# NVlabs/curobo

Measured on NVIDIA H100. Metric: rollout_cost_grad_evals_per_sec, higher is better.
Workload: dtype f32

## Files before the change

curobo_b200/csrc/cb200_kernels.cu:

```cuda
#include <cuda_runtime.h>
#include <stdio.h>
#include <stdlib.h>
#include <string.h>

#include <algorithm>
#include <cmath>
#include <vector>

#include "../../include/curobo_b200.h"
#include "cb200_blob.h"
#include "cb200_bspline.cuh"
#include "cb200_dynamics.cuh"
#include "cb200_dynamics_tile.cuh"
#include "cb200_launch.h"
#include "cb200_math.cuh"
#include "cb200_mesh.cuh"
#include "cb200_warp.cuh"

using namespace cb200;

namespace {

constexpr int kWarpsPerCta = 8;
#ifndef CB200_MINB
// ... 139 lines not shown
    bound_cost(qd, lim[d], lim[D + d], c.cspace_activation[0], wb[0], cost, gp);
    bound_cost(v, lim[2 * D + d], lim[3 * D + d], c.cspace_activation[1], wb[1], cost, gv);
    bound_cost(ac, lim[4 * D + d], lim[5 * D + d], c.cspace_activation[2], wb[2], cost, ga);
    bound_cost(jk, lim[6 * D + d], lim[7 * D + d], c.cspace_activation[3], wb[3], cost, gj);
    cspace_target_term(a, b, h, d, D, qd, cost, gp);
    l2_reg(v, wr[0], cost, gv);
    l2_reg(ac, wr[1], cost, ga);
    l2_reg(jk, wr[2], cost, gj);
    if (a.grad_vel) a.grad_vel[idx] = gv;
    if (a.grad_acc) a.grad_acc[idx] = ga;
    if (a.grad_jerk) a.grad_jerk[idx] = gj;
  }
  return cost;
}

template <bool SPLINE>
__device__ __forceinline__ void row_phase_a(const FusedArgs &a, const RobotView &rv, const EvalSmem &es, int lane, int e,
                                            int b, int h, float &cs_cost, float &pose_c) {
  const cb200_rollout_cfg &cfg = a.cfg;
  const int D = rv.D, S = rv.S, L = rv.L;
  cs_cost = 0.0f;
  #pragma unroll 1
  for (int d = lane; d < D; d += 32) {
    const bspline::State4 st = load_row_state<SPLINE>(a, e, b, h, d, D);
    es.qv[d] = st.p;
    float gp;
    const float c = cspace_dof(a, rv, e, b, h, d, st, gp);
    es.gqv[d] = gp;
    cs_cost += c;
    if (a.cspace_cost) a.cspace_cost[(size_t)e * D + d] = c;
  }
  __syncwarp();
  warp_fk(rv, es, lane);
  warp_spheres(rv, es, lane, a.robot_spheres ? reinterpret_cast<float4 *>(a.robot_spheres) + (size_t)e * S : nullptr,
               row_sphere_cfg(a, b, S));
  pose_c = 0.0f;
  const bool do_pose = (a.goal_position != nullptr);
  #pragma unroll 1
  for (int t = lane; t < L; t += 32) {
    const float *T = es.cumul + 12 * rv.tool_map[t];
    const V3 p = mk3(T[3], T[7], T[11]);
    const Q4 qt = quat_from_transform(T);
    if (a.link_pos) {
      float *o = a.link_pos + ((size_t)e * L + t) * 3;
      o[0] = p.x;
      o[1] = p.y;
      o[2] = p.z;
    }
    if (a.link_quat) *reinterpret_cast<float4 *>(a.link_quat + ((size_t)e * L + t) * 4) = make_float4(qt.w, qt.x, qt.y, qt.z);
    float *pg = es.pose_g + 8 * t;
    pg[0] = pg[1] = pg[2] = pg[4] = pg[5] = pg[6] = 0.0f;
    if (do_pose) {
      const int gi = a.idxs_goal ? __ldg(a.idxs_goal + b) : 0;
      const bool term = !(h < a.H - 1 && a.H > 1);
// ... 7 lines not shown
      const V3 om = quat_grad_to_omega(qt, po.gq_w, po.gq_x, po.gq_y, po.gq_z);
      pg[0] = po.g_pos.x;
      pg[1] = po.g_pos.y;
      pg[2] = po.g_pos.z;
      pg[4] = om.x;
      pg[5] = om.y;
      pg[6] = om.z;
      pose_c += po.pos_cost + po.rot_cost;
      if (a.pose_cost) {
        a.pose_cost[((size_t)e * L + t) * 2] = po.pos_cost;
        a.pose_cost[((size_t)e * L + t) * 2 + 1] = po.rot_cost;
      }
      if (a.pose_goalset_idx) a.pose_goalset_idx[(size_t)e * L + t] = po.goal_idx;
    }
  }
  __syncwarp();
}

struct RowB1 {
  float self_c, fmax, scene_c;
  int bi, bj, nnz;
};

template <bool SWEEP, int SCENE, bool CULL2 = true>
__device__ __forceinline__ RowB1 row_phase_b1(const FusedArgs &a, const RobotView &rv, const EvalSmem &es, int lane, int e,
                                              int b, const float4 *prev_sph, const float4 *next_sph) {
  const cb200_rollout_cfg &cfg = a.cfg;
  const int S = rv.S;
  RowB1 r{0.0f, 0.0f, 0.0f, 0, 0, 0};
  if (cfg.self_weight > 0.0f && rv.P > 0) {
    r.fmax = (rv.n_lp > 0) ? warp_self_collision_tiles<true, CULL2>(rv, es, lane, r.bi, r.bj)
                           : warp_self_collision_pairs(es.gsph, rv.pairs, rv.P, lane, r.bi, r.bj);
    r.self_c = (r.fmax > 0.0f) ? 0.5f * cfg.self_weight * r.fmax : 0.0f;
  }
  if (a.self_cost && lane == 0) a.self_cost[e] = r.self_c;
  __syncwarp();
  const bool do_scene = SCENE != 0 && cfg.scene_weight > 0.0f;
  const int env = (a.env_query_idx != nullptr) ? __ldg(a.env_query_idx + b) : 0;
  const float sdt = (SWEEP && cfg.use_speed_metric && (a.dt != nullptr || a.spl.knots != nullptr))
                        ? (a.spl.knots != nullptr ? __ldg(a.spl.traj_dt + __ldg(a.spl.goal_idx)) : __ldg(a.dt))
                        : 0.0f;
  int ce = 0, ncub = 0;
  bool cull = false;
  if ((SCENE & 1) && do_scene) {
    ce = env < a.cuboids.num_envs ? env : 0;
    ncub = a.cuboids.count[ce];
    if (ncub > a.cuboids.max_n) ncub = a.cuboids.max_n;
    cull = !SWEEP && rv.n_lp > 0 && ncub <= 32;
    if (cull) {
#pragma unroll 1
      for (int ca = lane; ca < rv.n_cl; ca += 32) {
        const float4 cb = rv.cl_bound_scene[ca];
        uint32_t mask = 0u;
        if (cb.w >= 0.0f) {
          const float *Tk = es.cumul + 12 * rv.cl_link[ca];
          const V3 cw = mk3(Tk[0] * cb.x + Tk[1] * cb.y + Tk[2] * cb.z + Tk[3], Tk[4] * cb.x + Tk[5] * cb.y + Tk[6] * cb.z + Tk[7],
                            Tk[8] * cb.x + Tk[9] * cb.y + Tk[10] * cb.z + Tk[11]);
#pragma unroll 1
          for (int i = 0; i < ncub; ++i) {
            const int kk = ce * a.cuboids.max_n + i;
            if (a.cuboids.enable[kk] != 1) continue;
            const ObsFrame f = load_obs_frame(a.cuboids.inv_pose + 8 * kk);
            const SdfGrad sg = cuboid_sdf_grad(to_obstacle(f, cw), ldgf(a.cuboids.dims + 4 * kk), ldgf(a.cuboids.dims + 4 * kk + 1),
                                               ldgf(a.cuboids.dims + 4 * kk + 2));
            if (sg.sdf < cb.w + cfg.scene_activation) mask |= (1u << i);
          }
        }
        es.cmask[ca] = mask;
      }
      __syncwarp();
    }
  }
#pragma unroll 1
  for (int s = lane; s < S; s += 32) {
    V3 g = mk3(0, 0, 0);
    float c = 0.0f;
    if (do_scene) {
      const float4 sp = es.sph[s];
      const V3 cen = mk3(sp.x, sp.y, sp.z);
      if (!SWEEP) {
        if (sp.w >= 0.0f) {
          if (SCENE & 1) {
            uint32_t m = cull ? es.cmask[rv.sph_cl[s]] : 0xffffffffu;
            const float radj = sp.w + cfg.scene_activation;
#pragma unroll 1
            for (int i = 0; i < ncub && m != 0u; ++i) {
              if (cull && !((m >> i) & 1u)) continue;
              if (cull) m &= ~(1u << i);
              const int kk = ce * a.cuboids.max_n + i;
// ... 23 lines not shown
        }
        if (next_sph != nullptr) {
          const float4 t = next_sph[s];
          nx = mk3(t.x, t.y, t.z);
        }
        c = sphere_scene_swept<SCENE>(cen, sp.w, cfg.scene_activation, cfg.scene_weight, prev_sph != nullptr, pv,
                                      next_sph != nullptr, nx, a.cuboids, a.voxels, env, g);
        if (cfg.use_speed_metric && prev_sph != nullptr && next_sph != nullptr) speed_metric(pv, cen, nx, sdt, c, g);
      }
    }
    es.gsph[s] = make_float4(g.x, g.y, g.z, 0.0f);
    r.nnz += (g.x != 0.0f || g.y != 0.0f || g.z != 0.0f) ? 1 : 0;
    r.scene_c += c;
    if (a.scene_cost) a.scene_cost[(size_t)e * S + s] = c;
  }
  __syncwarp();
  r.nnz = (int)__reduce_add_sync(kFull, (unsigned)r.nnz) + 2;
  return r;
}

template <bool SMALL = false>
__device__ __forceinline__ void row_phase_b2(const FusedArgs &a, const RobotView &rv, const EvalSmem &es,
                                             const unsigned char *smem_blob, int lane, int e, const RowB1 &r,
                                             float cs_cost, float pose_c) {
  if (r.fmax > 0.0f && lane == 0) {
    const float4 pi = es.sph[r.bi], pj = es.sph[r.bj];
    const float w = a.cfg.self_weight;
    float4 gi = es.gsph[r.bi], gj = es.gsph[r.bj];
    const float gx = w * (pj.x - pi.x), gy = w * (pj.y - pi.y), gz = w * (pj.z - pi.z);
    gi.x += gx;
    gi.y += gy;
    gi.z += gz;
    gj.x -= gx;
    gj.y -= gy;
    gj.z -= gz;
    es.gsph[r.bi] = gi;
    es.gsph[r.bj] = gj;
  }
  __syncwarp();
  float *gq = a.grad_q + (size_t)e * rv.D;
  if (!warp_fk_backward_sparse<SMALL>(rv, es, lane, gq, r.nnz)) warp_fk_backward_cold(smem_blob, a.blob, es.cumul, lane, gq);
  const float tot = warp_sum(cs_cost + pose_c + r.scene_c) + r.self_c;
  if (lane == 0) a.cost[e] = tot;
  __syncwarp();
}

#ifdef CB200_OOL_PHASES
struct PhaseAOut {
  float cs_cost, pose_c;
};
static __device__ __noinline__ PhaseAOut phase_a_ool(const FusedArgs *a, const unsigned char *smem, float *base, int lane,
                                                     int e, int b, int h) {
  const RobotView rv = make_robot_view(smem, a->blob);
  const EvalSmem es = carve_eval_smem(base, rv.nl, rv.D, rv.S, rv.L, rv.n_cl);
  PhaseAOut o;
  row_phase_a<false>(*a, rv, es, lane, e, b, h, o.cs_cost, o.pose_c);
  return o;
}
template <int SCENE>
static __device__ __noinline__ RowB1 phase_b1_ool(const FusedArgs *a, const unsigned char *smem, float *base, int lane, int e,
                                                  int b) {
  const RobotView rv = make_robot_view(smem, a->blob);
  const EvalSmem es = carve_eval_smem(base, rv.nl, rv.D, rv.S, rv.L, rv.n_cl);
  return row_phase_b1<false, SCENE>(*a, rv, es, lane, e, b, nullptr, nullptr);
}
static __device__ __noinline__ void phase_b2_ool(const FusedArgs *a, const unsigned char *smem, float *base, int lane, int e,
                                                 RowB1 r, float cs_cost, float pose_c) {
  const RobotView rv = make_robot_view(smem, a->blob);
  const EvalSmem es = carve_eval_smem(base, rv.nl, rv.D, rv.S, rv.L, rv.n_cl);
  row_phase_b2(*a, rv, es, smem, lane, e, r, cs_cost, pose_c);
}
#endif

template <int SCENE, bool SPLINE, int MINB = CB200_MINB>
__global__ void __launch_bounds__(kWarpsPerCta * 32, MINB) rollout_fused_kernel(const __grid_constant__ FusedArgs a) {
  CB200_EXTERN_SHARED __align__(128) unsigned char smem[];
  __shared__ unsigned long long mbar;
  stage_blob_to_smem(smem, a.blob, (uint32_t)a.blob_smem_bytes, &mbar);
  const int warp = threadIdx.x >> 5, lane = threadIdx.x & 31, nwarps = blockDim.x >> 5;
  float *base = reinterpret_cast<float *>(smem + a.blob_smem_bytes) + (size_t)warp * a.eval_floats;
  const int N = a.B * a.H;
  const int stride = gridDim.x * nwarps;
  int e = blockIdx.x * nwarps + warp;
  while (e < N) {
    int b = e, h = 0;
    if (a.H != 1) {
      b = e / a.H;
      h = e - b * a.H;
    }
#ifndef CB200_OOL_PHASES
    const RobotView rv = make_robot_view(smem, a.blob);
    const EvalSmem es = carve_eval_smem(base, rv.nl, rv.D, rv.S, rv.L, rv.n_cl);
    float cs_cost = 0.0f, pose_c = 0.0f;
    row_phase_a<SPLINE>(a, rv, es, lane, e, b, h, cs_cost, pose_c);
    const RowB1 r = row_phase_b1<false, SCENE, MINB != 3>(a, rv, es, lane, e, b, nullptr, nullptr);
    row_phase_b2<MINB == 3>(a, rv, es, smem, lane, e, r, cs_cost, pose_c);
#else
    const PhaseAOut pa = phase_a_ool(&a, smem, base, lane, e, b, h);
    const RowB1 r = phase_b1_ool<SCENE>(&a, smem, base, lane, e, b);
    phase_b2_ool(&a, smem, base, lane, e, r, pa.cs_cost, pa.pose_c);
#endif
    if (a.work_counter != nullptr) {
      int nxt = 0;
      if (lane == 0) nxt = stride + atomicAdd(a.work_counter, 1);
      e = __shfl_sync(kFull, nxt, 0);
    } else {
      e += stride;
    }
  }
  if (a.work_counter != nullptr && lane == 0) {
    __threadfence();
    if (atomicAdd(a.work_counter + 1, 1) == stride - 1) {
      a.work_counter[0] = 0;
      a.work_counter[1] = 0;
    }
  }
}

constexpr int kBigWarps = 16;

template <int SCENE, bool SMALL = false>
__device__ __forceinline__ RowB1 row_phase_b1_list(const FusedArgs &a, const RobotView &rv, const EvalSmem &es, int lane, int e,
                                                   int b, int &n_list, bool &dense) {
  const cb200_rollout_cfg &cfg = a.cfg;
  const int S = rv.S;
// ... 2780 lines not shown
            cand.nw = nw, cand.R = R, cand.per_sm = per_sm, cand.smem = need;
          }
        }
      }
      if (cand.nw == 0) return ret(cudaErrorInvalidConfiguration);
      cand.key = dkey;
      dpl = cand;
    }
    long long grid_ll = (long long)d.sm_count * dpl.per_sm;
    const long long need_ctas = (long long)io->batch_size * ((io->horizon + dpl.R - 1) / dpl.R);
    if (grid_ll > need_ctas) grid_ll = need_ctas;
    g_last_variant = CB200_VARIANT_TRAJ_DYN;
    CB200_LAUNCH(dk, (int)(grid_ll < 1 ? 1 : grid_ll), dpl.nw * 32, dpl.smem, (cudaStream_t)stream, a, dpl.R);
    return finish();
  }
  if (variant == 0 && arm_regcap != 0 && (scene <= 1 || arm_esdf != 0) && h.nl <= 24 && h.S <= 128) {
    kern = arm_table[scene];
    variant = 5;
  }
  const int minb = scene;
  struct Plan {
    long long key = -1;
    int nw = 0, per_sm = 0;
  };
  static thread_local Plan plans[6][4];
  Plan &pl = plans[variant][scene];
  const size_t halo_bytes = traj ? (size_t)2 * h.S * sizeof(float4) : 0;
  const long long key = ((long long)h.smem_bytes << 32) ^ ((long long)a.eval_floats << 8) ^ (long long)minb ^
                        (traj ? ((long long)io->horizon << 40) : 0) ^ ((long long)(d.ordinal + 1) << 56);
  if (key != pl.key) {
    cudaFuncAttributes fa;
    cudaError_t e0 = cudaFuncGetAttributes(&fa, kern);
    if (e0 != cudaSuccess) return ret(e0);
    const size_t limit = (size_t)d.max_smem - fa.sharedSizeBytes;
    const size_t max_need = (size_t)h.smem_bytes + halo_bytes + (size_t)kWarpsPerCta * a.eval_floats * sizeof(float);
    const size_t cap = std::min(max_need, limit);
    cudaError_t e = cudaFuncSetAttribute(kern, cudaFuncAttributeMaxDynamicSharedMemorySize, (int)cap);
    if (e != cudaSuccess) return ret(e);
    int best_nw = 0, best_per_sm = 0;
    double best_score = 0.0;
    static const int force_nw = []() {
      const char *e = getenv("CB200_FORCE_NW");
      return e ? atoi(e) : 0;
    }();
    for (int nw = kWarpsPerCta; nw >= 1; --nw) {
      if (force_nw > 0 && nw != force_nw) continue;
      const size_t need = (size_t)h.smem_bytes + halo_bytes + (size_t)nw * a.eval_floats * sizeof(float);
      if (need > limit) continue;
      int per_sm = 0;
      if (cudaOccupancyMaxActiveBlocksPerMultiprocessor(&per_sm, kern, nw * 32, need) != cudaSuccess) continue;
      double score = (double)per_sm * nw;
      if (traj) {
        const int tiles = (io->horizon + nw - 1) / nw;
        score *= (double)io->horizon / ((double)tiles * nw + 0.3 * 2.0 * (tiles - 1));
      }
      if (score > best_score) {
        best_score = score;
        best_nw = nw;
        best_per_sm = per_sm;
      }
    }
    if (best_nw == 0) return ret(cudaErrorInvalidConfiguration);
    pl.key = key;
    pl.nw = best_nw;
    pl.per_sm = best_per_sm;
  }
  const int nw = pl.nw;
  {
    const char *qs = getenv("CB200_QUEUE");
    a.work_counter = !(qs && atoi(qs) == 0) ? io->work_counter : nullptr;
    if (traj && (long long)io->batch_size * ((io->horizon + nw - 1) / nw) > 0x3fffffffLL) a.work_counter = nullptr;
  }
  const size_t smem = (size_t)h.smem_bytes + halo_bytes + (size_t)nw * a.eval_floats * sizeof(float);
  long long grid_ll = (long long)d.sm_count * pl.per_sm;
  const long long need_ctas = traj ? (long long)io->batch_size * ((io->horizon + nw - 1) / nw) : (N + nw - 1) / nw;
  if (grid_ll > need_ctas) grid_ll = need_ctas;
  const int grid = (int)(grid_ll < 1 ? 1 : grid_ll);
  if (need_ctas <= grid_ll) a.work_counter = nullptr;
  g_last_variant = traj ? CB200_VARIANT_TRAJ : (variant == 5 ? CB200_VARIANT_ARM : CB200_VARIANT_STANDARD);
  CB200_LAUNCH(kern, grid, nw * 32, smem, (cudaStream_t)stream, a);
  return finish();
}

}
```

curobo_b200/csrc/cb200_warp.cuh:

```cuda
#pragma once
#include "cb200_blob.h"
#include "cb200_math.cuh"

namespace cb200 {

constexpr unsigned kFull = 0xffffffffu;

struct RobotView {
  int nl, D, S, L, P, n_levels;
  const float *fixed;
  const float *joff;
  const int16_t *link_map;
  const int16_t *joint_map;
  const int8_t *joint_type;
  const int16_t *tool_map;
  const float4 *spheres;
  const int16_t *sph_link;
  const float *padding;
  const int16_t *link_sph_off;
  const int16_t *link_sph_idx;
  const int16_t *level_off;
  const int16_t *level_links;
  const unsigned long long *anc_mask;
  const int16_t *jl_off;
// ... 95 lines not shown
  EvalSmem e;
  e.cumul = base;
  e.sph = reinterpret_cast<float4 *>(base + nl * 12);
  e.gsph = nullptr;
  e.ft = base + nl * 12 + S * 4;
  e.bc = reinterpret_cast<float4 *>(e.ft + nl * 8);
  e.glist = e.bc + n_cl;
  e.contrib = reinterpret_cast<float *>(e.glist + kGradListCap);
  e.qv = e.contrib + nl;
  e.gqv = e.qv + D;
  e.pose_g = e.gqv + D;
  e.cmask = reinterpret_cast<uint32_t *>(e.pose_g + L * 8);
  return e;
}

__device__ __forceinline__ float warp_sum(float v) {
#pragma unroll
  for (int o = 16; o > 0; o >>= 1) v += __shfl_xor_sync(kFull, v, o);
  return v;
}

__device__ __forceinline__ void warp_fk_compose(const RobotView &rv, const EvalSmem &es, int lane);
__device__ __forceinline__ void warp_fk(const RobotView &rv, const EvalSmem &es, int lane) {
  const bool scratch = rv.S * 4 >= rv.nl * 12;
  float *loc = scratch ? reinterpret_cast<float *>(es.sph) : es.cumul;
  #pragma unroll 1
  for (int l = lane; l < rv.nl; l += 32) {
    int jt = rv.joint_type[l];
    float th = 0.0f;
    if (jt >= 0) th = rv.joff[2 * l] * es.qv[rv.joint_map[l]] + rv.joff[2 * l + 1];
    local_link_transform(rv.fixed + 12 * l, jt, th, (l == 0 ? es.cumul : loc) + 12 * l);
  }
  __syncwarp();
  warp_fk_compose(rv, es, lane);
}

__device__ __forceinline__ void warp_fk_compose(const RobotView &rv, const EvalSmem &es, int lane) {
  const bool scratch = rv.S * 4 >= rv.nl * 12;
  const float *loc = scratch ? reinterpret_cast<const float *>(es.sph) : es.cumul;
  const int sub = lane >> 4, k = lane & 15;
  const bool lane_ok = k < 12;
  const uint32_t row_off = (uint32_t)(k >> 2) * 16u, col_off = (uint32_t)(k & 3) * 4u, k_off = (uint32_t)k * 4u;
  const float cw = ((k & 3) == 3) ? 1.0f : 0.0f;
  unsigned char *cumb = reinterpret_cast<unsigned char *>(es.cumul);
  const unsigned char *locb = reinterpret_cast<const unsigned char *>(loc);
#pragma unroll 1
  for (int st = 0; st < rv.n_fk_steps; ++st) {
    const uint32_t w = rv.fk_sched[2 * st + sub];
    const uint32_t l_off = w & 0xffffu, p_off = w >> 16;
    const bool act = lane_ok && (l_off != 0xffffu);
    float out = 0.0f;
    if (act) {
      const float4 pr = *reinterpret_cast<const float4 *>(cumb + p_off + row_off);
      const float *Lm = reinterpret_cast<const float *>(locb + l_off + col_off);
      out = pr.x * Lm[0] + pr.y * Lm[4] + pr.z * Lm[8] + cw * pr.w;
    }
    if (!scratch) __syncwarp();
    if (act) *reinterpret_cast<float *>(cumb + l_off + k_off) = out;
    __syncwarp();
  }
}

__device__ __forceinline__ void warp_spheres(const RobotView &rv, const EvalSmem &es, int lane, float4 *out_global,
                                             const float4 *cfg_spheres = nullptr) {
  #pragma unroll 1
  for (int s = lane; s < rv.S; s += 32) {
    const float *T = es.cumul + 12 * rv.sph_link[s];
    const float4 p = cfg_spheres != nullptr ? __ldg(cfg_spheres + s) : rv.spheres[s];
    const float4 r0 = *reinterpret_cast<const float4 *>(T), r1 = *reinterpret_cast<const float4 *>(T + 4),
                 r2 = *reinterpret_cast<const float4 *>(T + 8);
    float4 w;
    w.x = r0.x * p.x + r0.y * p.y + r0.z * p.z + r0.w;
    w.y = r1.x * p.x + r1.y * p.y + r1.z * p.z + r1.w;
    w.z = r2.x * p.x + r2.y * p.y + r2.z * p.z + r2.w;
    w.w = p.w;
    es.sph[s] = w;
    if (out_global != nullptr) out_global[s] = w;
    if (es.gsph != nullptr) {
      w.w = p.w + rv.padding[s];
      es.gsph[s] = w;
    }
  }
}

__device__ __forceinline__ float warp_self_collision_pairs(const float4 *psph, const uint32_t *pairs, int P, int lane,
                                                           int &bi, int &bj) {
  float best = 0.0f;
  uint32_t best_p = 0xffffffffu;
  #pragma unroll 1
  for (int p = lane; p < P; p += 32) {
    const uint32_t pr = __ldg(pairs + p);
    const float4 a = psph[pr & 0xffffu], b = psph[pr >> 16];
    const float rs = a.w + b.w;
    const float dx = a.x - b.x, dy = a.y - b.y, dz = a.z - b.z;
    float f = rs * rs - (dx * dx + dy * dy + dz * dz);
    if (!(a.w >= 0.0f && b.w >= 0.0f)) f = 0.0f;
    if (f > best) {
      best = f;
      best_p = (uint32_t)p;
    }
  }
  const uint32_t fb = __reduce_max_sync(kFull, __float_as_uint(best));
  const uint32_t cand = (__float_as_uint(best) == fb && best > 0.0f) ? best_p : 0xffffffffu;
  const uint32_t win = __reduce_min_sync(kFull, cand);
  bi = bj = 0;
  if (win == 0xffffffffu) return 0.0f;
  const uint32_t pr = __ldg(pairs + win);
  bi = (int)(pr & 0xffffu);
  bj = (int)(pr >> 16);
  return __uint_as_float(fb);
}

template <bool PADDED_COPY>
__device__ __forceinline__ float4 padded_sphere(const RobotView &rv, const EvalSmem &es, int i) {
  if (PADDED_COPY) return es.gsph[i];
  float4 x = es.sph[i];
  x.w += rv.padding[i];
  return x;
}

template <bool PADDED_COPY = true, bool CULL2 = true>
__device__ __forceinline__ float warp_self_collision_tiles(const RobotView &rv, const EvalSmem &es, int lane, int &bi,
                                                           int &bj, int base0 = 0, int stride = 32,
                                                           unsigned char *idx_scratch = nullptr,
                                                           unsigned long long *key_out = nullptr, bool fill_bounds = true) {
  if (fill_bounds) {
    #pragma unroll 1
    for (int a = lane; a < rv.n_cl; a += 32) {
      const float4 c = rv.cl_bound[a];
      const float *T = es.cumul + 12 * rv.cl_link[a];
      es.bc[a] = make_float4(T[0] * c.x + T[1] * c.y + T[2] * c.z + T[3], T[4] * c.x + T[5] * c.y + T[6] * c.z + T[7],
                             T[8] * c.x + T[9] * c.y + T[10] * c.z + T[11], c.w);
    }
    __syncwarp();
  }
  unsigned long long key = 0ull;
  #pragma unroll 1
  for (int base = base0; base < rv.n_lp; base += stride) {
    uint32_t pr = 0;
    bool hit = false;
    if (base + lane < rv.n_lp) {
      pr = rv.lp[base + lane];
      const float4 A = es.bc[pr & 0xffffu], B = es.bc[pr >> 16];
      const float dx = A.x - B.x, dy = A.y - B.y, dz = A.z - B.z, rs = A.w + B.w;
      hit = (A.w >= 0.0f) && (B.w >= 0.0f) && (dx * dx + dy * dy + dz * dz < rs * rs);
    }
    unsigned m = __ballot_sync(kFull, hit);
    while (m) {
      const int src = __ffs(m) - 1;
      m &= m - 1;
      const uint32_t q = __shfl_sync(kFull, pr, src);
      const int a = q & 0xffffu, b = q >> 16;
      const int sa = rv.cl_start[a], na = rv.cl_start[a + 1] - sa;
      const int sb = rv.cl_start[b], nb = rv.cl_start[b + 1] - sb;
      if (CULL2 && es.ft != nullptr && na <= 32 && nb <= 32 && na * nb > 64) {
        const float4 A = es.bc[a], B = es.bc[b];
        bool ca = false, cb = false;
        if (lane < na) {
          const float4 x = padded_sphere<PADDED_COPY>(rv, es, sa + lane);
          const float dx = x.x - B.x, dy = x.y - B.y, dz = x.z - B.z, rs = x.w + B.w;
          ca = (x.w >= 0.0f) && (dx * dx + dy * dy + dz * dz < rs * rs);
        }
        if (lane < nb) {
          const float4 y = padded_sphere<PADDED_COPY>(rv, es, sb + lane);
          const float dx = y.x - A.x, dy = y.y - A.y, dz = y.z - A.z, rs = y.w + A.w;
          cb = (y.w >= 0.0f) && (dx * dx + dy * dy + dz * dz < rs * rs);
// ... 14 lines not shown
          const float4 x = padded_sphere<PADDED_COPY>(rv, es, i), y = padded_sphere<PADDED_COPY>(rv, es, j);
          const float rs = x.w + y.w;
          const float dx = x.x - y.x, dy = x.y - y.y, dz = x.z - y.z;
          const float f = rs * rs - (dx * dx + dy * dy + dz * dz);
          if (f > 0.0f) {
            const unsigned long long k = ((unsigned long long)__float_as_uint(f) << 32) |
                                         ((unsigned long long)(0xffffu - (unsigned)i) << 16) | (0xffffu - (unsigned)j);
            key = k > key ? k : key;
          }
        }
        __syncwarp();
        continue;
      }
      const float inv_nb = 1.0f / (float)nb;
      #pragma unroll 1
      for (int t = lane; t < na * nb; t += 32) {
        const int io = (int)(((float)t + 0.5f) * inv_nb);
        const int i = sa + io, j = sb + (t - io * nb);
        const float4 x = padded_sphere<PADDED_COPY>(rv, es, i), y = padded_sphere<PADDED_COPY>(rv, es, j);
        const float rs = x.w + y.w;
        const float dx = x.x - y.x, dy = x.y - y.y, dz = x.z - y.z;
        const float f = rs * rs - (dx * dx + dy * dy + dz * dz);
        if (f > 0.0f && x.w >= 0.0f && y.w >= 0.0f) {
          const unsigned long long k = ((unsigned long long)__float_as_uint(f) << 32) |
                                       ((unsigned long long)(0xffffu - (unsigned)i) << 16) | (0xffffu - (unsigned)j);
          key = k > key ? k : key;
        }
      }
    }
  }
#pragma unroll
  for (int o = 16; o > 0; o >>= 1) {
    const unsigned long long other = __shfl_xor_sync(kFull, key, o);
    key = other > key ? other : key;
  }
  if (key_out != nullptr) *key_out = key;
  bi = bj = 0;
  if (key == 0ull) return 0.0f;
  bi = 0xffff - (int)((key >> 16) & 0xffffu);
  bj = 0xffff - (int)(key & 0xffffu);
  return __uint_as_float((uint32_t)(key >> 32));
}

__device__ __forceinline__ void warp_fk_upsweep(const RobotView &rv, const EvalSmem &es, int lane, float *gq_out);
__device__ __forceinline__ void warp_fk_backward(const RobotView &rv, const EvalSmem &es, int lane, float *gq_out) {
  #pragma unroll 1
  for (int k = lane; k < rv.nl; k += 32) {
    const float *Tk = es.cumul + 12 * k;
    const V3 o = mk3(Tk[3], Tk[7], Tk[11]);
    V3 F = mk3(0, 0, 0), T = mk3(0, 0, 0);
    #pragma unroll 1
    for (int i = rv.link_sph_off[k]; i < rv.link_sph_off[k + 1]; ++i) {
      const int s = rv.link_sph_idx[i];
      const float4 g4 = es.gsph[s];
      const V3 g = mk3(g4.x, g4.y, g4.z);
      if (g.x == 0.0f && g.y == 0.0f && g.z == 0.0f) continue;
      const float4 p4 = es.sph[s];
      F = F + g;
      T = T + cross(mk3(p4.x, p4.y, p4.z) - o, g);
    }
    for (int e = 0; e < rv.L; ++e) {
      if (rv.tool_map[e] != k) continue;
      F = F + mk3(es.pose_g[8 * e + 0], es.pose_g[8 * e + 1], es.pose_g[8 * e + 2]);
      T = T + mk3(es.pose_g[8 * e + 4], es.pose_g[8 * e + 5], es.pose_g[8 * e + 6]);
    }
    float *ft = es.ft + 8 * k;
    ft[0] = F.x;
    ft[1] = F.y;
    ft[2] = F.z;
    ft[4] = T.x;
    ft[5] = T.y;
    ft[6] = T.z;
  }
  __syncwarp();
  warp_fk_upsweep(rv, es, lane, gq_out);
}

__device__ __forceinline__ void warp_fk_upsweep(const RobotView &rv, const EvalSmem &es, int lane, float *gq_out) {
  #pragma unroll 1
  for (int j = lane; j < rv.nl; j += 32) {
    const int jt = rv.joint_type[j];
    float res = 0.0f;
    if (jt >= 0) {
      const float *Tj = es.cumul + 12 * j;
      const V3 oj = mk3(Tj[3], Tj[7], Tj[11]);
      V3 F = mk3(0, 0, 0), T = mk3(0, 0, 0);
      #pragma unroll 1
      for (int k = j; k < rv.nl; ++k) {
        if (!((rv.anc_mask[k] >> j) & 1ull)) continue;
        const float *ft = es.ft + 8 * k;
        const V3 Fk = mk3(ft[0], ft[1], ft[2]);
        const float *Tk = es.cumul + 12 * k;
        const V3 ok = mk3(Tk[3], Tk[7], Tk[11]);
        F = F + Fk;
        T = T + mk3(ft[4], ft[5], ft[6]) + cross(ok - oj, Fk);
      }
      const int ax = (jt >= JT_XR) ? jt - JT_XR : jt;
      const V3 a = mk3(Tj[ax], Tj[4 + ax], Tj[8 + ax]);
      res = rv.joff[2 * j] * ((jt >= JT_XR) ? dot(a, T) : dot(a, F));
    }
    es.contrib[j] = res;
  }
  __syncwarp();
  for (int d = lane; d < rv.D; d += 32) {
    float g = es.gqv[d];
    for (int i = rv.jl_off[d]; i < rv.jl_off[d + 1]; ++i) g += es.contrib[rv.jl_idx[i]];
    gq_out[d] = g;
  }
}

static __device__ __noinline__ void warp_fk_backward_cold(const unsigned char *smem_blob, const unsigned char *gmem_blob,
                                                          float *eval_base, int lane, float *gq_out) {
  const RobotView rv = make_robot_view(smem_blob, gmem_blob);
  const EvalSmem es = carve_eval_smem(eval_base, rv.nl, rv.D, rv.S, rv.L, rv.n_cl);
  warp_fk_backward(rv, es, lane, gq_out);
}

template <bool SMALL = false>
__device__ __forceinline__ bool warp_fk_backward_sparse(const RobotView &rv, const EvalSmem &es, int lane, float *gq_out,
                                                        int nnz) {
  if (nnz > 2 * rv.nl) return false;
  if (SMALL) {
    float sc = 0.0f;
    V3 ax = mk3(0, 0, 0), og = mk3(0, 0, 0);
    int jt = -1;
    if (lane < rv.nl) {
      jt = rv.joint_type[lane];
      if (jt >= 0) {
        const float *Tj = es.cumul + 12 * lane;
        const int a = (jt >= JT_XR) ? jt - JT_XR : jt;
        ax = mk3(Tj[a], Tj[4 + a], Tj[8 + a]);
        og = mk3(Tj[3], Tj[7], Tj[11]);
        sc = rv.joff[2 * lane];
      }
    }
    float acc = 0.0f;
    const int n_entries = rv.S + rv.L;
#pragma unroll 1
    for (int base = 0; base < n_entries; base += 32) {
      const int s = base + lane;
      bool nz = false;
      if (s < rv.S) {
        const float4 g = es.gsph[s];
        nz = (g.x != 0.0f) || (g.y != 0.0f) || (g.z != 0.0f);
      } else if (s < n_entries) {
        const float *pg = es.pose_g + 8 * (s - rv.S);
        nz = pg[0] != 0.0f || pg[1] != 0.0f || pg[2] != 0.0f || pg[4] != 0.0f || pg[5] != 0.0f || pg[6] != 0.0f;
      }
      unsigned m = __ballot_sync(kFull, nz);
      while (m) {
        const int ss = base + __ffs(m) - 1;
        m &= m - 1;
        V3 p, g, om = mk3(0, 0, 0);
        int k;
        if (ss < rv.S) {
          const float4 g4 = es.gsph[ss], p4 = es.sph[ss];
          k = rv.sph_link[ss];
          p = mk3(p4.x, p4.y, p4.z);
          g = mk3(g4.x, g4.y, g4.z);
        } else {
          const float *pg = es.pose_g + 8 * (ss - rv.S);
          k = rv.tool_map[ss - rv.S];
          const float *Tk = es.cumul + 12 * k;
          p = mk3(Tk[3], Tk[7], Tk[11]);
          g = mk3(pg[0], pg[1], pg[2]);
          om = mk3(pg[4], pg[5], pg[6]);
        }
        if (jt >= 0 && ((rv.anc_mask[k] >> lane) & 1ull))
          acc += (jt >= JT_XR) ? sc * (dot(ax, cross(p - og, g)) + dot(ax, om)) : sc * dot(ax, g);
      }
    }
    if (lane < rv.nl) es.contrib[lane] = acc;
    __syncwarp();
    for (int d = lane; d < rv.D; d += 32) {
      float g = es.gqv[d];
      for (int i = rv.jl_off[d]; i < rv.jl_off[d + 1]; ++i) g += es.contrib[rv.jl_idx[i]];
      gq_out[d] = g;
    }
    return true;
  }
  const int nu = rv.nl > 32 ? 2 : 1;
  V3 ax[2], og[2];
  float sc[2];
  int jt[2];
#pragma unroll
  for (int u = 0; u < 2; ++u) {
    const int j = lane + 32 * u;
    jt[u] = -1;
    if (u >= nu) continue;
// ... 302 lines not shown
```

Measured before the change: 226.7 million.

## Process two rollout rows per warp using half-warp rows in arm kernel

```diff
diff --git a/curobo_b200/csrc/cb200_kernels.cu b/curobo_b200/csrc/cb200_kernels.cu
--- a/curobo_b200/csrc/cb200_kernels.cu
+++ b/curobo_b200/csrc/cb200_kernels.cu
@@ -177,14 +177,14 @@
   return cost;
 }
 
-template <bool SPLINE>
+template <bool SPLINE, int W = 32>
 __device__ __forceinline__ void row_phase_a(const FusedArgs &a, const RobotView &rv, const EvalSmem &es, int lane, int e,
                                             int b, int h, float &cs_cost, float &pose_c) {
   const cb200_rollout_cfg &cfg = a.cfg;
   const int D = rv.D, S = rv.S, L = rv.L;
   cs_cost = 0.0f;
   #pragma unroll 1
-  for (int d = lane; d < D; d += 32) {
+  for (int d = lane; d < D; d += W) {
     const bspline::State4 st = load_row_state<SPLINE>(a, e, b, h, d, D);
     es.qv[d] = st.p;
     float gp;
@@ -193,14 +193,14 @@
     cs_cost += c;
     if (a.cspace_cost) a.cspace_cost[(size_t)e * D + d] = c;
   }
-  __syncwarp();
-  warp_fk(rv, es, lane);
-  warp_spheres(rv, es, lane, a.robot_spheres ? reinterpret_cast<float4 *>(a.robot_spheres) + (size_t)e * S : nullptr,
-               row_sphere_cfg(a, b, S));
+  row_sync<W>();
+  warp_fk<W>(rv, es, lane);
+  warp_spheres<W>(rv, es, lane, a.robot_spheres ? reinterpret_cast<float4 *>(a.robot_spheres) + (size_t)e * S : nullptr,
+                  row_sphere_cfg(a, b, S));
   pose_c = 0.0f;
   const bool do_pose = (a.goal_position != nullptr);
   #pragma unroll 1
-  for (int t = lane; t < L; t += 32) {
+  for (int t = lane; t < L; t += W) {
     const float *T = es.cumul + 12 * rv.tool_map[t];
     const V3 p = mk3(T[3], T[7], T[11]);
     const Q4 qt = quat_from_transform(T);
@@ -238,7 +238,7 @@
       if (a.pose_goalset_idx) a.pose_goalset_idx[(size_t)e * L + t] = po.goal_idx;
     }
   }
-  __syncwarp();
+  row_sync<W>();
 }
 
 struct RowB1 {
@@ -246,19 +246,19 @@
   int bi, bj, nnz;
 };
 
-template <bool SWEEP, int SCENE, bool CULL2 = true>
+template <bool SWEEP, int SCENE, bool CULL2 = true, int W = 32>
 __device__ __forceinline__ RowB1 row_phase_b1(const FusedArgs &a, const RobotView &rv, const EvalSmem &es, int lane, int e,
                                               int b, const float4 *prev_sph, const float4 *next_sph) {
   const cb200_rollout_cfg &cfg = a.cfg;
   const int S = rv.S;
   RowB1 r{0.0f, 0.0f, 0.0f, 0, 0, 0};
   if (cfg.self_weight > 0.0f && rv.P > 0) {
-    r.fmax = (rv.n_lp > 0) ? warp_self_collision_tiles<true, CULL2>(rv, es, lane, r.bi, r.bj)
-                           : warp_self_collision_pairs(es.gsph, rv.pairs, rv.P, lane, r.bi, r.bj);
+    r.fmax = (rv.n_lp > 0) ? warp_self_collision_tiles<true, CULL2, W>(rv, es, lane, r.bi, r.bj)
+                           : warp_self_collision_pairs<W>(es.gsph, rv.pairs, rv.P, lane, r.bi, r.bj);
     r.self_c = (r.fmax > 0.0f) ? 0.5f * cfg.self_weight * r.fmax : 0.0f;
   }
   if (a.self_cost && lane == 0) a.self_cost[e] = r.self_c;
-  __syncwarp();
+  row_sync<W>();
   const bool do_scene = SCENE != 0 && cfg.scene_weight > 0.0f;
   const int env = (a.env_query_idx != nullptr) ? __ldg(a.env_query_idx + b) : 0;
   const float sdt = (SWEEP && cfg.use_speed_metric && (a.dt != nullptr || a.spl.knots != nullptr))
@@ -273,7 +273,7 @@
     cull = !SWEEP && rv.n_lp > 0 && ncub <= 32;
     if (cull) {
 #pragma unroll 1
-      for (int ca = lane; ca < rv.n_cl; ca += 32) {
+      for (int ca = lane; ca < rv.n_cl; ca += W) {
         const float4 cb = rv.cl_bound_scene[ca];
         uint32_t mask = 0u;
         if (cb.w >= 0.0f) {
@@ -292,11 +292,11 @@
         }
         es.cmask[ca] = mask;
       }
-      __syncwarp();
+      row_sync<W>();
     }
   }
 #pragma unroll 1
-  for (int s = lane; s < S; s += 32) {
+  for (int s = lane; s < S; s += W) {
     V3 g = mk3(0, 0, 0);
     float c = 0.0f;
     if (do_scene) {
@@ -350,12 +350,12 @@
     r.scene_c += c;
     if (a.scene_cost) a.scene_cost[(size_t)e * S + s] = c;
   }
-  __syncwarp();
-  r.nnz = (int)__reduce_add_sync(kFull, (unsigned)r.nnz) + 2;
+  row_sync<W>();
+  r.nnz = (int)row_reduce<W, 0>((unsigned)r.nnz) + 2;
   return r;
 }
 
-template <bool SMALL = false>
+template <bool SMALL = false, int W = 32>
 __device__ __forceinline__ void row_phase_b2(const FusedArgs &a, const RobotView &rv, const EvalSmem &es,
                                              const unsigned char *smem_blob, int lane, int e, const RowB1 &r,
                                              float cs_cost, float pose_c) {
@@ -373,78 +373,87 @@
     es.gsph[r.bi] = gi;
     es.gsph[r.bj] = gj;
   }
-  __syncwarp();
+  row_sync<W>();
   float *gq = a.grad_q + (size_t)e * rv.D;
-  if (!warp_fk_backward_sparse<SMALL>(rv, es, lane, gq, r.nnz)) warp_fk_backward_cold(smem_blob, a.blob, es.cumul, lane, gq);
-  const float tot = warp_sum(cs_cost + pose_c + r.scene_c) + r.self_c;
+  if (!warp_fk_backward_sparse<SMALL, W>(rv, es, lane, gq, r.nnz)) warp_fk_backward_cold<W>(smem_blob, a.blob, es.cumul, lane, gq);
+  const float tot = warp_sum<W>(cs_cost + pose_c + r.scene_c) + r.self_c;
   if (lane == 0) a.cost[e] = tot;
-  __syncwarp();
+  row_sync<W>();
 }
 
 #ifdef CB200_OOL_PHASES
 struct PhaseAOut {
   float cs_cost, pose_c;
 };
+template <int W>
 static __device__ __noinline__ PhaseAOut phase_a_ool(const FusedArgs *a, const unsigned char *smem, float *base, int lane,
                                                      int e, int b, int h) {
   const RobotView rv = make_robot_view(smem, a->blob);
   const EvalSmem es = carve_eval_smem(base, rv.nl, rv.D, rv.S, rv.L, rv.n_cl);
   PhaseAOut o;
-  row_phase_a<false>(*a, rv, es, lane, e, b, h, o.cs_cost, o.pose_c);
+  row_phase_a<false, W>(*a, rv, es, lane, e, b, h, o.cs_cost, o.pose_c);
   return o;
 }
-template <int SCENE>
+template <int SCENE, int W>
 static __device__ __noinline__ RowB1 phase_b1_ool(const FusedArgs *a, const unsigned char *smem, float *base, int lane, int e,
                                                   int b) {
   const RobotView rv = make_robot_view(smem, a->blob);
   const EvalSmem es = carve_eval_smem(base, rv.nl, rv.D, rv.S, rv.L, rv.n_cl);
-  return row_phase_b1<false, SCENE>(*a, rv, es, lane, e, b, nullptr, nullptr);
-}
+  return row_phase_b1<false, SCENE, W == 32, W>(*a, rv, es, lane, e, b, nullptr, nullptr);
+}
+template <int W>
 static __device__ __noinline__ void phase_b2_ool(const FusedArgs *a, const unsigned char *smem, float *base, int lane, int e,
                                                  RowB1 r, float cs_cost, float pose_c) {
   const RobotView rv = make_robot_view(smem, a->blob);
   const EvalSmem es = carve_eval_smem(base, rv.nl, rv.D, rv.S, rv.L, rv.n_cl);
-  row_phase_b2(*a, rv, es, smem, lane, e, r, cs_cost, pose_c);
+  row_phase_b2<W == 16, W>(*a, rv, es, smem, lane, e, r, cs_cost, pose_c);
 }
 #endif
 
-template <int SCENE, bool SPLINE, int MINB = CB200_MINB>
+template <int SCENE, bool SPLINE, int MINB = CB200_MINB, int ROWS = 1>
 __global__ void __launch_bounds__(kWarpsPerCta * 32, MINB) rollout_fused_kernel(const __grid_constant__ FusedArgs a) {
+  static_assert(ROWS == 1 || (ROWS == 2 && MINB == 3 && !SPLINE), "paired rows: arm build only");
+  constexpr int W = 32 / ROWS;
   CB200_EXTERN_SHARED __align__(128) unsigned char smem[];
   __shared__ unsigned long long mbar;
   stage_blob_to_smem(smem, a.blob, (uint32_t)a.blob_smem_bytes, &mbar);
-  const int warp = threadIdx.x >> 5, lane = threadIdx.x & 31, nwarps = blockDim.x >> 5;
-  float *base = reinterpret_cast<float *>(smem + a.blob_smem_bytes) + (size_t)warp * a.eval_floats;
+  const int warp = threadIdx.x >> 5, lane = threadIdx.x & (W - 1), nwarps = blockDim.x >> 5;
+  const int half = ROWS == 1 ? 0 : (int)(threadIdx.x >> 4) & 1;
+  const bool leader = (threadIdx.x & 31) == 0;
+  float *base = reinterpret_cast<float *>(smem + a.blob_smem_bytes) + (size_t)(warp * ROWS + half) * a.eval_floats;
   const int N = a.B * a.H;
   const int stride = gridDim.x * nwarps;
-  int e = blockIdx.x * nwarps + warp;
-  while (e < N) {
-    int b = e, h = 0;
-    if (a.H != 1) {
-      b = e / a.H;
-      h = e - b * a.H;
-    }
+  int u = blockIdx.x * nwarps + warp;
+  while (u * ROWS < N) {
+    const int e = u * ROWS + half;
+    if (ROWS == 1 || e < N) {
+      int b = e, h = 0;
+      if (a.H != 1) {
+        b = e / a.H;
+        h = e - b * a.H;
+      }
 #ifndef CB200_OOL_PHASES
-    const RobotView rv = make_robot_view(smem, a.blob);
-    const EvalSmem es = carve_eval_smem(base, rv.nl, rv.D, rv.S, rv.L, rv.n_cl);
-    float cs_cost = 0.0f, pose_c = 0.0f;
-    row_phase_a<SPLINE>(a, rv, es, lane, e, b, h, cs_cost, pose_c);
-    const RowB1 r = row_phase_b1<false, SCENE, MINB != 3>(a, rv, es, lane, e, b, nullptr, nullptr);
-    row_phase_b2<MINB == 3>(a, rv, es, smem, lane, e, r, cs_cost, pose_c);
+      const RobotView rv = make_robot_view(smem, a.blob);
+      const EvalSmem es = carve_eval_smem(base, rv.nl, rv.D, rv.S, rv.L, rv.n_cl);
+      float cs_cost = 0.0f, pose_c = 0.0f;
+      row_phase_a<SPLINE, W>(a, rv, es, lane, e, b, h, cs_cost, pose_c);
+      const RowB1 r = row_phase_b1<false, SCENE, MINB != 3, W>(a, rv, es, lane, e, b, nullptr, nullptr);
+      row_phase_b2<MINB == 3, W>(a, rv, es, smem, lane, e, r, cs_cost, pose_c);
 #else
-    const PhaseAOut pa = phase_a_ool(&a, smem, base, lane, e, b, h);
-    const RowB1 r = phase_b1_ool<SCENE>(&a, smem, base, lane, e, b);
-    phase_b2_ool(&a, smem, base, lane, e, r, pa.cs_cost, pa.pose_c);
+      const PhaseAOut pa = phase_a_ool<W>(&a, smem, base, lane, e, b, h);
+      const RowB1 r = phase_b1_ool<SCENE, W>(&a, smem, base, lane, e, b);
+      phase_b2_ool<W>(&a, smem, base, lane, e, r, pa.cs_cost, pa.pose_c);
 #endif
+    }
     if (a.work_counter != nullptr) {
       int nxt = 0;
-      if (lane == 0) nxt = stride + atomicAdd(a.work_counter, 1);
-      e = __shfl_sync(kFull, nxt, 0);
+      if (leader) nxt = stride + atomicAdd(a.work_counter, 1);
+      u = __shfl_sync(kFull, nxt, 0);
     } else {
-      e += stride;
-    }
-  }
-  if (a.work_counter != nullptr && lane == 0) {
+      u += stride;
+    }
+  }
+  if (a.work_counter != nullptr && leader) {
     __threadfence();
     if (atomicAdd(a.work_counter + 1, 1) == stride - 1) {
       a.work_counter[0] = 0;
@@ -3255,26 +3264,34 @@
     CB200_LAUNCH(dk, (int)(grid_ll < 1 ? 1 : grid_ll), dpl.nw * 32, dpl.smem, (cudaStream_t)stream, a, dpl.R);
     return finish();
   }
+  int rows_per_warp = 1;
   if (variant == 0 && arm_regcap != 0 && (scene <= 1 || arm_esdf != 0) && h.nl <= 24 && h.S <= 128) {
-    kern = arm_table[scene];
-    variant = 5;
-  }
+    const char *ps = getenv("CB200_ARM_PAIRS");
+    const int pairs_env = ps ? atoi(ps) : -1;
+    const bool pairs = h.nl <= 16 && (scene & 2) == 0 &&
+                       (pairs_env >= 0 ? pairs_env != 0 : 2LL * N >= 3LL * d.sm_count * 3 * kWarpsPerCta);
+    static KernelT const arm_pairs_table[2] = {rollout_fused_kernel<0, false, 3, 2>, rollout_fused_kernel<1, false, 3, 2>};
+    kern = pairs ? arm_pairs_table[scene] : arm_table[scene];
+    rows_per_warp = pairs ? 2 : 1;
+    variant = pairs ? 6 : 5;
+  }
+  const int warp_floats = rows_per_warp * a.eval_floats;
   const int minb = scene;
   struct Plan {
     long long key = -1;
     int nw = 0, per_sm = 0;
   };
-  static thread_local Plan plans[6][4];
+  static thread_local Plan plans[7][4];
   Plan &pl = plans[variant][scene];
   const size_t halo_bytes = traj ? (size_t)2 * h.S * sizeof(float4) : 0;
-  const long long key = ((long long)h.smem_bytes << 32) ^ ((long long)a.eval_floats << 8) ^ (long long)minb ^
+  const long long key = ((long long)h.smem_bytes << 32) ^ ((long long)warp_floats << 8) ^ (long long)minb ^
                         (traj ? ((long long)io->horizon << 40) : 0) ^ ((long long)(d.ordinal + 1) << 56);
   if (key != pl.key) {
     cudaFuncAttributes fa;
     cudaError_t e0 = cudaFuncGetAttributes(&fa, kern);
     if (e0 != cudaSuccess) return ret(e0);
     const size_t limit = (size_t)d.max_smem - fa.sharedSizeBytes;
-    const size_t max_need = (size_t)h.smem_bytes + halo_bytes + (size_t)kWarpsPerCta * a.eval_floats * sizeof(float);
+    const size_t max_need = (size_t)h.smem_bytes + halo_bytes + (size_t)kWarpsPerCta * warp_floats * sizeof(float);
     const size_t cap = std::min(max_need, limit);
     cudaError_t e = cudaFuncSetAttribute(kern, cudaFuncAttributeMaxDynamicSharedMemorySize, (int)cap);
     if (e != cudaSuccess) return ret(e);
@@ -3286,7 +3303,7 @@
     }();
     for (int nw = kWarpsPerCta; nw >= 1; --nw) {
       if (force_nw > 0 && nw != force_nw) continue;
-      const size_t need = (size_t)h.smem_bytes + halo_bytes + (size_t)nw * a.eval_floats * sizeof(float);
+      const size_t need = (size_t)h.smem_bytes + halo_bytes + (size_t)nw * warp_floats * sizeof(float);
       if (need > limit) continue;
       int per_sm = 0;
       if (cudaOccupancyMaxActiveBlocksPerMultiprocessor(&per_sm, kern, nw * 32, need) != cudaSuccess) continue;
@@ -3312,13 +3329,14 @@
     a.work_counter = !(qs && atoi(qs) == 0) ? io->work_counter : nullptr;
     if (traj && (long long)io->batch_size * ((io->horizon + nw - 1) / nw) > 0x3fffffffLL) a.work_counter = nullptr;
   }
-  const size_t smem = (size_t)h.smem_bytes + halo_bytes + (size_t)nw * a.eval_floats * sizeof(float);
+  const size_t smem = (size_t)h.smem_bytes + halo_bytes + (size_t)nw * warp_floats * sizeof(float);
   long long grid_ll = (long long)d.sm_count * pl.per_sm;
-  const long long need_ctas = traj ? (long long)io->batch_size * ((io->horizon + nw - 1) / nw) : (N + nw - 1) / nw;
+  const long long units = (N + rows_per_warp - 1) / rows_per_warp;
+  const long long need_ctas = traj ? (long long)io->batch_size * ((io->horizon + nw - 1) / nw) : (units + nw - 1) / nw;
   if (grid_ll > need_ctas) grid_ll = need_ctas;
   const int grid = (int)(grid_ll < 1 ? 1 : grid_ll);
   if (need_ctas <= grid_ll) a.work_counter = nullptr;
-  g_last_variant = traj ? CB200_VARIANT_TRAJ : (variant == 5 ? CB200_VARIANT_ARM : CB200_VARIANT_STANDARD);
+  g_last_variant = traj ? CB200_VARIANT_TRAJ : (variant >= 5 ? CB200_VARIANT_ARM : CB200_VARIANT_STANDARD);
   CB200_LAUNCH(kern, grid, nw * 32, smem, (cudaStream_t)stream, a);
   return finish();
 }
diff --git a/curobo_b200/csrc/cb200_warp.cuh b/curobo_b200/csrc/cb200_warp.cuh
--- a/curobo_b200/csrc/cb200_warp.cuh
+++ b/curobo_b200/csrc/cb200_warp.cuh
@@ -133,31 +133,119 @@
   return e;
 }
 
+template <int W>
+__device__ __forceinline__ unsigned row_mask() {
+  static_assert(W == 32 || W == 16, "a row is a warp or a half-warp");
+  return W == 32 ? kFull : 0xffffu << (threadIdx.x & 16u);
+}
+#ifdef CB200_SIMT_EMULATION
+template <class T, class F>
+inline T half_exchange(T v, F pick) {
+  static unsigned long long slot[16 * 16];
+  const int t = threadIdx.x;
+  unsigned long long bits = 0;
+  std::memcpy(&bits, &v, sizeof(T));
+  slot[t] = bits;
+  simt::named_barrier(t >> 4, 16);
+  const unsigned long long got = pick(slot + (t & ~15));
+  simt::named_barrier(t >> 4, 16);
+  T r;
+  std::memcpy(&r, &got, sizeof(T));
+  return r;
+}
+#endif
+template <int W>
+__device__ __forceinline__ void row_sync() {
+  if (W == 32) {
+    __syncwarp();
+  } else {
+#ifdef CB200_SIMT_EMULATION
+    simt::named_barrier(threadIdx.x >> 4, 16);
+#else
+    __syncwarp(row_mask<W>());
+#endif
+  }
+}
+template <int W>
+__device__ __forceinline__ unsigned row_ballot(bool p) {
+  if (W == 32) return __ballot_sync(kFull, p);
+#ifdef CB200_SIMT_EMULATION
+  return half_exchange((unsigned)p, [](const unsigned long long *s) {
+    unsigned long long m = 0;
+    for (int i = 0; i < 16; ++i) m |= (s[i] & 1ull) << i;
+    return m;
+  });
+#else
+  const unsigned m = row_mask<W>();
+  return (__ballot_sync(m, p) & m) >> (threadIdx.x & 16u);
+#endif
+}
+template <int W>
+__device__ __forceinline__ uint32_t row_shfl(uint32_t v, int src) {
+  if (W == 32) return __shfl_sync(kFull, v, src);
+#ifdef CB200_SIMT_EMULATION
+  return half_exchange(v, [src](const unsigned long long *s) { return s[src & 15]; });
+#else
+  return __shfl_sync(row_mask<W>(), v, src, W);
+#endif
+}
+template <int W, class T>
+__device__ __forceinline__ T row_shfl_xor(T v, int o) {
+  if (W == 32) return __shfl_xor_sync(kFull, v, o);
+#ifdef CB200_SIMT_EMULATION
+  const int me = threadIdx.x & 15;
+  return half_exchange(v, [me, o](const unsigned long long *s) { return s[me ^ o]; });
+#else
+  return __shfl_xor_sync(row_mask<W>(), v, o);
+#endif
+}
+template <int W, int OP>
+__device__ __forceinline__ unsigned row_reduce(unsigned v) {
+  if (W == 32) return OP == 0 ? __reduce_add_sync(kFull, v) : OP == 1 ? __reduce_min_sync(kFull, v) : __reduce_max_sync(kFull, v);
+#ifdef CB200_SIMT_EMULATION
+  return half_exchange(v, [](const unsigned long long *s) {
+    unsigned r = (unsigned)s[0];
+    for (int i = 1; i < 16; ++i) {
+      const unsigned x = (unsigned)s[i];
+      r = OP == 0 ? r + x : OP == 1 ? (x < r ? x : r) : (x > r ? x : r);
+    }
+    return (unsigned long long)r;
+  });
+#else
+  const unsigned m = row_mask<W>();
+  return OP == 0 ? __reduce_add_sync(m, v) : OP == 1 ? __reduce_min_sync(m, v) : __reduce_max_sync(m, v);
+#endif
+}
+
+template <int W = 32>
 __device__ __forceinline__ float warp_sum(float v) {
 #pragma unroll
-  for (int o = 16; o > 0; o >>= 1) v += __shfl_xor_sync(kFull, v, o);
+  for (int o = W / 2; o > 0; o >>= 1) v += row_shfl_xor<W>(v, o);
   return v;
 }
 
+template <int W = 32>
 __device__ __forceinline__ void warp_fk_compose(const RobotView &rv, const EvalSmem &es, int lane);
+template <int W = 32>
 __device__ __forceinline__ void warp_fk(const RobotView &rv, const EvalSmem &es, int lane) {
   const bool scratch = rv.S * 4 >= rv.nl * 12;
   float *loc = scratch ? reinterpret_cast<float *>(es.sph) : es.cumul;
   #pragma unroll 1
-  for (int l = lane; l < rv.nl; l += 32) {
+  for (int l = lane; l < rv.nl; l += W) {
     int jt = rv.joint_type[l];
     float th = 0.0f;
     if (jt >= 0) th = rv.joff[2 * l] * es.qv[rv.joint_map[l]] + rv.joff[2 * l + 1];
     local_link_transform(rv.fixed + 12 * l, jt, th, (l == 0 ? es.cumul : loc) + 12 * l);
   }
-  __syncwarp();
-  warp_fk_compose(rv, es, lane);
-}
-
+  row_sync<W>();
+  warp_fk_compose<W>(rv, es, lane);
+}
+
+template <int W>
 __device__ __forceinline__ void warp_fk_compose(const RobotView &rv, const EvalSmem &es, int lane) {
   const bool scratch = rv.S * 4 >= rv.nl * 12;
   const float *loc = scratch ? reinterpret_cast<const float *>(es.sph) : es.cumul;
-  const int sub = lane >> 4, k = lane & 15;
+  const int half = lane >> 4, k = lane & 15;
   const bool lane_ok = k < 12;
   const uint32_t row_off = (uint32_t)(k >> 2) * 16u, col_off = (uint32_t)(k & 3) * 4u, k_off = (uint32_t)k * 4u;
   const float cw = ((k & 3) == 3) ? 1.0f : 0.0f;
@@ -165,25 +253,31 @@
   const unsigned char *locb = reinterpret_cast<const unsigned char *>(loc);
 #pragma unroll 1
   for (int st = 0; st < rv.n_fk_steps; ++st) {
-    const uint32_t w = rv.fk_sched[2 * st + sub];
-    const uint32_t l_off = w & 0xffffu, p_off = w >> 16;
-    const bool act = lane_ok && (l_off != 0xffffu);
-    float out = 0.0f;
-    if (act) {
-      const float4 pr = *reinterpret_cast<const float4 *>(cumb + p_off + row_off);
-      const float *Lm = reinterpret_cast<const float *>(locb + l_off + col_off);
-      out = pr.x * Lm[0] + pr.y * Lm[4] + pr.z * Lm[8] + cw * pr.w;
-    }
-    if (!scratch) __syncwarp();
-    if (act) *reinterpret_cast<float *>(cumb + l_off + k_off) = out;
-    __syncwarp();
-  }
-}
-
+#pragma unroll
+    for (int pass = 0; pass < 32 / W; ++pass) {
+      const int sub = W == 32 ? half : pass;
+      const uint32_t w = rv.fk_sched[2 * st + sub];
+      const uint32_t l_off = w & 0xffffu, p_off = w >> 16;
+      if (W == 16 && l_off == 0xffffu) continue;
+      const bool act = lane_ok && (l_off != 0xffffu);
+      float out = 0.0f;
+      if (act) {
+        const float4 pr = *reinterpret_cast<const float4 *>(cumb + p_off + row_off);
+        const float *Lm = reinterpret_cast<const float *>(locb + l_off + col_off);
+        out = pr.x * Lm[0] + pr.y * Lm[4] + pr.z * Lm[8] + cw * pr.w;
+      }
+      if (!scratch) row_sync<W>();
+      if (act) *reinterpret_cast<float *>(cumb + l_off + k_off) = out;
+      row_sync<W>();
+    }
+  }
+}
+
+template <int W = 32>
 __device__ __forceinline__ void warp_spheres(const RobotView &rv, const EvalSmem &es, int lane, float4 *out_global,
                                              const float4 *cfg_spheres = nullptr) {
   #pragma unroll 1
-  for (int s = lane; s < rv.S; s += 32) {
+  for (int s = lane; s < rv.S; s += W) {
     const float *T = es.cumul + 12 * rv.sph_link[s];
     const float4 p = cfg_spheres != nullptr ? __ldg(cfg_spheres + s) : rv.spheres[s];
     const float4 r0 = *reinterpret_cast<const float4 *>(T), r1 = *reinterpret_cast<const float4 *>(T + 4),
@@ -202,12 +296,13 @@
   }
 }
 
+template <int W = 32>
 __device__ __forceinline__ float warp_self_collision_pairs(const float4 *psph, const uint32_t *pairs, int P, int lane,
                                                            int &bi, int &bj) {
   float best = 0.0f;
   uint32_t best_p = 0xffffffffu;
   #pragma unroll 1
-  for (int p = lane; p < P; p += 32) {
+  for (int p = lane; p < P; p += W) {
     const uint32_t pr = __ldg(pairs + p);
     const float4 a = psph[pr & 0xffffu], b = psph[pr >> 16];
     const float rs = a.w + b.w;
@@ -219,9 +314,9 @@
       best_p = (uint32_t)p;
     }
   }
-  const uint32_t fb = __reduce_max_sync(kFull, __float_as_uint(best));
+  const uint32_t fb = row_reduce<W, 2>(__float_as_uint(best));
   const uint32_t cand = (__float_as_uint(best) == fb && best > 0.0f) ? best_p : 0xffffffffu;
-  const uint32_t win = __reduce_min_sync(kFull, cand);
+  const uint32_t win = row_reduce<W, 1>(cand);
   bi = bj = 0;
   if (win == 0xffffffffu) return 0.0f;
   const uint32_t pr = __ldg(pairs + win);
@@ -238,20 +333,21 @@
   return x;
 }
 
-template <bool PADDED_COPY = true, bool CULL2 = true>
+template <bool PADDED_COPY = true, bool CULL2 = true, int W = 32>
 __device__ __forceinline__ float warp_self_collision_tiles(const RobotView &rv, const EvalSmem &es, int lane, int &bi,
-                                                           int &bj, int base0 = 0, int stride = 32,
+                                                           int &bj, int base0 = 0, int stride = W,
                                                            unsigned char *idx_scratch = nullptr,
                                                            unsigned long long *key_out = nullptr, bool fill_bounds = true) {
+  static_assert(W == 32 || !CULL2, "the second-level cull is written for whole-warp rows");
   if (fill_bounds) {
     #pragma unroll 1
-    for (int a = lane; a < rv.n_cl; a += 32) {
+    for (int a = lane; a < rv.n_cl; a += W) {
       const float4 c = rv.cl_bound[a];
       const float *T = es.cumul + 12 * rv.cl_link[a];
       es.bc[a] = make_float4(T[0] * c.x + T[1] * c.y + T[2] * c.z + T[3], T[4] * c.x + T[5] * c.y + T[6] * c.z + T[7],
                              T[8] * c.x + T[9] * c.y + T[10] * c.z + T[11], c.w);
     }
-    __syncwarp();
+    row_sync<W>();
   }
   unsigned long long key = 0ull;
   #pragma unroll 1
@@ -264,11 +360,11 @@
       const float dx = A.x - B.x, dy = A.y - B.y, dz = A.z - B.z, rs = A.w + B.w;
       hit = (A.w >= 0.0f) && (B.w >= 0.0f) && (dx * dx + dy * dy + dz * dz < rs * rs);
     }
-    unsigned m = __ballot_sync(kFull, hit);
+    unsigned m = row_ballot<W>(hit);
     while (m) {
       const int src = __ffs(m) - 1;
       m &= m - 1;
-      const uint32_t q = __shfl_sync(kFull, pr, src);
+      const uint32_t q = row_shfl<W>(pr, src);
       const int a = q & 0xffffu, b = q >> 16;
       const int sa = rv.cl_start[a], na = rv.cl_start[a + 1] - sa;
       const int sb = rv.cl_start[b], nb = rv.cl_start[b + 1] - sb;
@@ -313,7 +409,7 @@
       }
       const float inv_nb = 1.0f / (float)nb;
       #pragma unroll 1
-      for (int t = lane; t < na * nb; t += 32) {
+      for (int t = lane; t < na * nb; t += W) {
         const int io = (int)(((float)t + 0.5f) * inv_nb);
         const int i = sa + io, j = sb + (t - io * nb);
         const float4 x = padded_sphere<PADDED_COPY>(rv, es, i), y = padded_sphere<PADDED_COPY>(rv, es, j);
@@ -329,8 +425,8 @@
     }
   }
 #pragma unroll
-  for (int o = 16; o > 0; o >>= 1) {
-    const unsigned long long other = __shfl_xor_sync(kFull, key, o);
+  for (int o = W / 2; o > 0; o >>= 1) {
+    const unsigned long long other = row_shfl_xor<W>(key, o);
     key = other > key ? other : key;
   }
   if (key_out != nullptr) *key_out = key;
@@ -341,10 +437,12 @@
   return __uint_as_float((uint32_t)(key >> 32));
 }
 
+template <int W = 32>
 __device__ __forceinline__ void warp_fk_upsweep(const RobotView &rv, const EvalSmem &es, int lane, float *gq_out);
+template <int W = 32>
 __device__ __forceinline__ void warp_fk_backward(const RobotView &rv, const EvalSmem &es, int lane, float *gq_out) {
   #pragma unroll 1
-  for (int k = lane; k < rv.nl; k += 32) {
+  for (int k = lane; k < rv.nl; k += W) {
     const float *Tk = es.cumul + 12 * k;
     const V3 o = mk3(Tk[3], Tk[7], Tk[11]);
     V3 F = mk3(0, 0, 0), T = mk3(0, 0, 0);
@@ -371,13 +469,14 @@
     ft[5] = T.y;
     ft[6] = T.z;
   }
-  __syncwarp();
-  warp_fk_upsweep(rv, es, lane, gq_out);
-}
-
+  row_sync<W>();
+  warp_fk_upsweep<W>(rv, es, lane, gq_out);
+}
+
+template <int W>
 __device__ __forceinline__ void warp_fk_upsweep(const RobotView &rv, const EvalSmem &es, int lane, float *gq_out) {
   #pragma unroll 1
-  for (int j = lane; j < rv.nl; j += 32) {
+  for (int j = lane; j < rv.nl; j += W) {
     const int jt = rv.joint_type[j];
     float res = 0.0f;
     if (jt >= 0) {
@@ -400,24 +499,26 @@
     }
     es.contrib[j] = res;
   }
-  __syncwarp();
-  for (int d = lane; d < rv.D; d += 32) {
+  row_sync<W>();
+  for (int d = lane; d < rv.D; d += W) {
     float g = es.gqv[d];
     for (int i = rv.jl_off[d]; i < rv.jl_off[d + 1]; ++i) g += es.contrib[rv.jl_idx[i]];
     gq_out[d] = g;
   }
 }
 
+template <int W = 32>
 static __device__ __noinline__ void warp_fk_backward_cold(const unsigned char *smem_blob, const unsigned char *gmem_blob,
                                                           float *eval_base, int lane, float *gq_out) {
   const RobotView rv = make_robot_view(smem_blob, gmem_blob);
   const EvalSmem es = carve_eval_smem(eval_base, rv.nl, rv.D, rv.S, rv.L, rv.n_cl);
-  warp_fk_backward(rv, es, lane, gq_out);
-}
-
-template <bool SMALL = false>
+  warp_fk_backward<W>(rv, es, lane, gq_out);
+}
+
+template <bool SMALL = false, int W = 32>
 __device__ __forceinline__ bool warp_fk_backward_sparse(const RobotView &rv, const EvalSmem &es, int lane, float *gq_out,
                                                         int nnz) {
+  static_assert(W == 32 || SMALL, "half-warp rows take the one-link-per-lane form");
   if (nnz > 2 * rv.nl) return false;
   if (SMALL) {
     float sc = 0.0f;
@@ -436,7 +537,7 @@
     float acc = 0.0f;
     const int n_entries = rv.S + rv.L;
 #pragma unroll 1
-    for (int base = 0; base < n_entries; base += 32) {
+    for (int base = 0; base < n_entries; base += W) {
       const int s = base + lane;
       bool nz = false;
       if (s < rv.S) {
@@ -446,7 +547,7 @@
         const float *pg = es.pose_g + 8 * (s - rv.S);
         nz = pg[0] != 0.0f || pg[1] != 0.0f || pg[2] != 0.0f || pg[4] != 0.0f || pg[5] != 0.0f || pg[6] != 0.0f;
       }
-      unsigned m = __ballot_sync(kFull, nz);
+      unsigned m = row_ballot<W>(nz);
       while (m) {
         const int ss = base + __ffs(m) - 1;
         m &= m - 1;
@@ -470,8 +571,8 @@
       }
     }
     if (lane < rv.nl) es.contrib[lane] = acc;
-    __syncwarp();
-    for (int d = lane; d < rv.D; d += 32) {
+    row_sync<W>();
+    for (int d = lane; d < rv.D; d += W) {
       float g = es.gqv[d];
       for (int i = rv.jl_off[d]; i < rv.jl_off[d + 1]; ++i) g += es.contrib[rv.jl_idx[i]];
       gq_out[d] = g;
```

Result: faster. 261.7 million, median of 6 (+15.4%).
